# pennneutrinos/chroma

Hardware: AMD Instinct MI355X
Metric: photons/sec (propagate_hit) (higher is better)
Workload: dtype f32

## Files before the change

### chroma_amd/csrc/chroma_hip.hip

```cpp
#include <math.h>
#include <stdio.h>
#include <stdlib.h>
#include <string.h>
#include <algorithm>

#ifndef CHROMA_EXPERIMENTAL
#define CHROMA_EXPERIMENTAL 0
#endif
#ifndef CHROMA_HYBRID_RENDER
#define CHROMA_HYBRID_RENDER 1
#endif
#include "chroma_internal.h"
#include "propagate_device.h"

#include "kernel_propagate_fused.h"

#include "kernel_step_control.h"

#include "kernels_raycast_crosscheck.h"

#include "kernel_raycast_quad.h"

#include "kernel_raycast_pair.h"

// ... 60 lines not shown
    {"pair", nullptr, Cast::PAIR, 32, 4 * PAIR_WAVES_PER_EU, "CHROMA_PAIR_WAVES_PER_CU", PAIR_STACK + COOP_SPILL, SPILL_COOP, CHROMA_WALK_QUAD, false, true},
    {"literal", "exact", Cast::LITERAL, 16, 4 * QUAD_WAVES_PER_EU, "CHROMA_QUAD_WAVES_PER_CU", 0, SPILL_COOP, -1, true, true},
    {"literal_lane", nullptr, Cast::LITERAL_LANE, PROP_BLOCK, 20, "CHROMA_RAY_WAVES_PER_CU", 0, SPILL_NONE, -1, false, false},
};
static const int NWALKS = sizeof WALKS / sizeof WALKS[0];
static_assert(NWALKS == CHROMA_WALK_LITERAL_LANE + 1, "one row per CHROMA_WALK_*");

static bool walk_fits(const Walk &w, const chroma_geometry *geom)
{
    return w.stack == 0 || (geom->view.wnodes != nullptr && geom->wide_stack_need <= w.stack);
}

struct CallPlan {
    int tail_mode;
    bool counting;
    Cast cast;
    bool chain;
    bool tail_watch;
    bool tail;
    bool isect_quad;
    unsigned spill;
    int packet;
    int autosort;
};

static int make_plan(const CallState &cs, const chroma_geometry *geom, int walk, int tail, int counting, CallPlan *plan)
{
    if (walk >= NWALKS) return set_error(CHROMA_ERR_INVALID, "unknown walk mode %d", walk);
    if (tail > CHROMA_TAIL_FUSED) return set_error(CHROMA_ERR_INVALID, "unknown tail mode %d", tail);
    const int w = walk >= 0 ? walk : cs.walk;
    CallPlan p = {};
    p.tail_mode = tail >= 0 ? tail : cs.tail_mode;
    p.counting = counting >= 0 ? counting != 0 : cs.counting != 0;
    int r = w;
    while (!walk_fits(WALKS[r], geom)) {
        r = WALKS[r].fallback;
        if (w == CHROMA_WALK_PAIR && r == CHROMA_WALK_COOP) r = WALKS[r].fallback;
    }
    p.cast = WALKS[r].cast;
    p.chain = r == w && WALKS[w].chain;
    const bool fits_coop = walk_fits(WALKS[CHROMA_WALK_COOP], geom);
    p.tail_watch = p.tail_mode == CHROMA_TAIL_COOP && WALKS[w].tail;
    p.tail = p.tail_watch && fits_coop;
    p.isect_quad = fits_coop && WALKS[w].stack != 0;
    if (p.tail_mode != CHROMA_TAIL_FUSED) p.spill = WALKS[r].spill | (p.tail ? SPILL_COOP : SPILL_NONE);
    if (p.chain && p.cast == Cast::QUAD) {
        p.autosort = cs.autosort_mode;
#if CHROMA_EXPERIMENTAL
        if (geom->wide_stack_need <= PACKET_STACK) p.packet = cs.packet_mode;
#endif
    }
    *plan = p;
    return CHROMA_OK;
}

static int ensure_spill(const CallScope &scope, unsigned kinds)
{
    chroma_ctx *ctx = scope.ctx; CallState &cs = scope.state();
    const struct { SpillKind kind; uint2 **buf; size_t depth; } bufs[] = {{SPILL_COOP, &cs.coop_spill, COOP_SPILL},
                                                                          {SPILL_WIDE, &cs.wide_spill, WIDE_SPILL}};
    for (const auto &b : bufs) {
        if (!(kinds & b.kind) || *b.buf) continue;
        size_t rays = 0;
        for (const Walk &w : WALKS)
            if (w.spill == b.kind) rays = std::max(rays, (size_t)ctx->waves[(int)w.cast] * w.rays_per_wave);
        HIP_TRY(hipSetDevice(ctx->device));
        HIP_TRY(ctx_malloc(ctx, (void **)b.buf, rays * b.depth * sizeof(uint2)));
    }
    return CHROMA_OK;
}

static unsigned cast_waves(const chroma_ctx *ctx, Cast cast, long long n)
{
    const long long per = WALKS[(int)cast].rays_per_wave;
    return (unsigned)std::min<long long>((n + per - 1) / per, ctx->waves[(int)cast]);
}
// ... 54 lines not shown
namespace {
struct PropagateCall {
    const CallScope &scope; CallState &cs;
    chroma_ctx *ctx; chroma_geometry *geom;
    CallPlan plan;
    PhotonView pv; chroma_rng rng; chroma_propagate_options opt;
    uint64_t nphotons; uint32_t ncopies;
    uint32_t *in_q, *out_q;
    float4 *work_in, *work_out;
    float4 *rays, *rays_next;
    float4 *final_rec;
    uint32_t final_epoch;
    HitsOut ho;
    bool finalize;
    chroma_propagate_stats acc;
    long long n_upper;
    bool finalized;
    chroma_tracks *tracks;

    hipEvent_t *events(int step) const { return opt.time_kernels ? cs.step_events.data() + EV_PER_STEP * step : nullptr; }

    int load_working()
    {
        const unsigned blocks = (unsigned)std::min<uint64_t>((nphotons + PHYS_BLOCK - 1) / PHYS_BLOCK, (uint64_t)ctx->physics_blocks);
        int rc = scope.clear_words(W_PACKET_USE, W_PACKET_END - W_PACKET_USE); if (rc) return rc;
        uint32_t *d_order = nullptr;
        rc = propagate_order(*this, &d_order); if (rc) return rc;
        hipLaunchKernelGGL(k_load_working, dim3(blocks), dim3(PHYS_BLOCK), 0, ctx->stream, geom->view, pv, in_q, work_in,
                           (uint64_t)nphotons, ncopies, (uint32_t)(nphotons / ncopies), plan.chain ? rays : nullptr,
                           plan.packet == 2 ? cs.d_words + W_PACKET_COHERENT : nullptr, (const uint32_t *)d_order, plan.cast == Cast::LITERAL ? 1 : 0);
        if (d_order) { chroma_free(ctx, d_order); acc.reordered += nphotons; }
#if CHROMA_EXPERIMENTAL
        if (plan.packet)
            hipLaunchKernelGGL(k_packet_decide, dim3(1), dim3(1), 0, ctx->stream, cs.d_words + W_PACKET_COHERENT, cs.d_words + W_PACKET_USE,
                               (uint64_t)nphotons, plan.packet);
#endif
        HIP_TRY(hipGetLastError());
        return CHROMA_OK;
    }

    void launch_step_begin(uint32_t first_n)
    {
        hipLaunchKernelGGL(k_step_begin, dim3(1), dim3(1), 0, ctx->stream, in_q, out_q, cs.d_step,
                           tracks ? 0u : opt.use_weights ? 0xFFFFFFFFu : (uint32_t)(PROP_BLOCK * 16 * 8), first_n);
    }

    void launch_physics(int scatter_first, int fixup)
    {
        StepState *st = cs.d_step;
        float4 *chained = plan.chain ? rays_next : nullptr;
        const bool plain = geom->view.plain_optics != 0;
        bool deal = false;
#if PHYS_DEAL
        deal = plain && !final_rec;
#endif
        const int pb = deal ? PHYS_DEAL_BLOCK : PHYS_BLOCK_OF(!plain);
        unsigned blocks = (unsigned)std::min<long long>((n_upper + pb - 1) / pb, std::max<long long>(1, (long long)ctx->physics_blocks * PHYS_BLOCK / pb));
        if (fixup == 1 && plain) blocks = std::max(std::min(blocks, 64u), blocks / 8);
        DeviceCounters *pc = plan.counting ? cs.d_counters : nullptr;
#if PHYS_DEAL
        if (deal) {
            hipLaunchKernelGGL(k_physics_deal, dim3(blocks), dim3(PHYS_DEAL_BLOCK), 0, ctx->stream, geom->view, pv, st, work_in, out_q, work_out,
                               cs.hit_triangle, cs.hit_distance, rng.seed, rng.photon_id_base, opt.use_weights, scatter_first,
                               cs.retry_list, fixup, pc, chained);
            return;
        }
#endif
        const int literal_rays = fixup == 2 ? 1 : 0;
        with_bool(!plain, [&](auto FULL) {
            hipLaunchKernelGGL((k_physics<FULL>), dim3(blocks), dim3(PHYS_BLOCK_OF(FULL)), 0, ctx->stream, geom->view, pv, st, work_in, out_q,
                               work_out, cs.hit_triangle, cs.hit_distance, rng.seed, rng.photon_id_base, opt.use_weights, scatter_first,
                               cs.retry_list, fixup, pc, chained, final_rec, final_epoch, literal_rays);
        });
    }

    int launch_split_step(int scatter_first, hipEvent_t *ev, uint32_t first_n, bool packet)
    {
        if (n_upper <= 0) return CHROMA_OK;
        StepState *st = cs.d_step;
        const Cast cast = plan.cast;
        const bool exact = cast == Cast::LITERAL || cast == Cast::LITERAL_LANE;
        const dim3 block(PROP_BLOCK);
        auto record = [&](int slot) { return ev ? hipEventRecord(ev[slot], ctx->stream) : hipSuccess; };
        const unsigned rblocks = (unsigned)std::min<long long>((n_upper + PROP_BLOCK - 1) / PROP_BLOCK, 8 * 256);
        auto retry = [&](auto C) {
            hipLaunchKernelGGL((k_raycast_retry<C>), dim3(rblocks), block, 0, ctx->stream, geom->view, rays, st, cs.hit_triangle,
                               cs.hit_distance, cs.retry_list, cs.d_counters);
        };
        launch_step_begin(first_n);
        HIP_TRY(record(EV_STEP_BEGIN));
        if (!plan.chain) {
            unsigned sblocks = (unsigned)std::min<long long>((n_upper + 255) / 256, (long long)ctx->physics_blocks * 4);
            hipLaunchKernelGGL(k_ray_setup, dim3(sblocks), dim3(256), 0, ctx->stream, geom->view, work_in, st, rays,
                               cs.hit_triangle, cs.hit_distance, cs.retry_list, &st->retry, cast == Cast::LITERAL ? 1 : 0);
        }
        HIP_TRY(record(EV_PACKET_BEGIN));
        const uint32_t *skip_quad = nullptr;
#if CHROMA_EXPERIMENTAL
        if (packet) {
// ... 26 lines not shown
                                   cs.hit_distance, cs.retry_list, cs.coop_spill, cs.d_counters, ctx->coop_chunk);
                break;
            case Cast::WIDE:
                hipLaunchKernelGGL((k_raycast_wide<C>), grid, block, 0, ctx->stream, geom->view, rays, 0, st, cs.hit_triangle,
                                   cs.hit_distance, cs.retry_list, cs.wide_spill, cs.d_counters, ctx->ray_chunk);
                break;
            case Cast::PERSISTENT:
                hipLaunchKernelGGL((k_raycast_persistent<C>), grid, block, 0, ctx->stream, geom->view, rays, 0, st, cs.hit_triangle,
                                   cs.hit_distance, cs.retry_list, cs.d_counters);
                break;
            case Cast::LITERAL:
                hipLaunchKernelGGL((k_raycast_literal<C>), grid, block, 0, ctx->stream, geom->view, rays, st, cs.hit_triangle,
                                   cs.hit_distance, cs.coop_spill, cs.d_counters, ctx->coop_chunk, chained, cs.retry_list,
                                   ctx->claim_static);
                retry(C);
                break;
            case Cast::LITERAL_LANE:
                hipLaunchKernelGGL((k_raycast_retry<C, true>), grid, block, 0, ctx->stream, geom->view, rays, st, cs.hit_triangle,
                                   cs.hit_distance, cs.retry_list, cs.d_counters);
                break;
            }
        });
        HIP_TRY(record(EV_CAST_END));
        launch_physics(scatter_first, exact ? 2 : 0);
        HIP_TRY(record(EV_PHYSICS_END));
        if (!exact) {
            with_bool(plan.counting, retry);
            launch_physics(scatter_first, 1);
        }
        HIP_TRY(record(EV_STEP_END));
        HIP_TRY(hipGetLastError());
        if (plan.chain) std::swap(rays, rays_next);
        return CHROMA_OK;
    }

    int launch_tail(int nsteps, int scatter_first, hipEvent_t *ev, uint32_t first_n, bool *done)
    {
        *done = false;
        const unsigned waves = cast_waves(ctx, Cast::COOP, n_upper);
        if ((long long)waves * 8 < n_upper) return CHROMA_OK;
        launch_step_begin(first_n);
        HitsOut beside; memset(&beside, 0, sizeof beside);
        uint32_t *words = nullptr;
        if (finalize) {
            beside = ho;
            words = cs.d_words;
            int rc = scope.clear_results(); if (rc) return rc;
            if (final_rec)
                hipLaunchKernelGGL(k_mark_tail, dim3(32), dim3(256), 0, ctx->stream, in_q, final_rec, photon_tail_stamp(final_epoch));
            HIP_TRY(hipEventRecord(cs.ev_fork, ctx->stream));
        }
// ... 46 lines not shown
        }
        return CHROMA_OK;
    }

    int run_device_steps()
    {
        const int max_steps = opt.max_steps;
        HIP_TRY(hipMemsetAsync(cs.d_step, 0, sizeof(StepState), ctx->stream));
        hipLaunchKernelGGL(k_set_word, dim3(1), dim3(1), 0, ctx->stream, in_q, 1u);
        hipLaunchKernelGGL(k_set_word, dim3(1), dim3(1), 0, ctx->stream, out_q, 1u);
        int rc = load_working(); if (rc) return rc;
        const int nev = opt.time_kernels ? EV_PER_STEP * max_steps : 0;
        while ((int)cs.step_events.size() < nev) { hipEvent_t e; HIP_TRY(hipEventCreate(&e)); cs.step_events.push_back(e); }
        const long long few = (long long)PROP_BLOCK * 16 * 8;
        int step = 0, next_check = 1, tail_step = -1;
        bool done = false;
        while (step < max_steps && !done) {
            const int scatter_first = step == 0 ? opt.scatter_first : 0;
            const uint32_t first_n = step == 0 ? (uint32_t)nphotons : 0u;
            if (plan.tail && n_upper < few) {
                rc = launch_tail(max_steps - step, scatter_first, events(step), first_n, &done); if (rc) return rc;
                if (done) { tail_step = step++; break; }
            }
            rc = launch_split_step(scatter_first, events(step), first_n, step == 0 && plan.packet != 0); if (rc) return rc;
            step++;
            std::swap(in_q, out_q);
            std::swap(work_in, work_out);
            if (step == next_check && step < max_steps) {
                rc = scope.read_survivors(in_q, &n_upper); if (rc) return rc;
                if (n_upper <= 0) done = true;
                next_check = (plan.tail_watch && n_upper < 16 * few) ? step + 1 : (step < 8) ? step * 2 : step + 8;
            }
        }
        if (!done) {
            unsigned blocks = (unsigned)std::min<long long>((n_upper + 255) / 256, 4096);
            hipLaunchKernelGGL(k_store_working, dim3(std::max(blocks, 1u)), dim3(256), 0, ctx->stream, geom->view, pv, in_q, work_in);
        }
        HIP_TRY(hipMemcpyAsync(cs.h_step, cs.d_step, sizeof(StepState), hipMemcpyDeviceToHost, ctx->stream));
        HIP_TRY(hipStreamSynchronize(ctx->stream));
        acc.launches += ((const StepState *)cs.h_step)->launches;
        return opt.time_kernels ? read_step_times(step, tail_step) : CHROMA_OK;
    }

    void store_working()
    {
        const unsigned blocks = (unsigned)std::min<long long>((n_upper + 255) / 256, 4096);
        hipLaunchKernelGGL(k_store_working, dim3(std::max(blocks, 1u)), dim3(256), 0, ctx->stream, geom->view, pv, in_q, work_in);
// ... 137 lines not shown

int propagate_settings(const CallScope &scope)
{
    chroma_ctx *ctx = scope.ctx; CallState &cs = scope.state();
    hipDeviceProp_t prop;
    HIP_TRY(hipGetDeviceProperties(&prop, ctx->device));
    ctx->physics_blocks = prop.multiProcessorCount * 8;
    const char *walk = getenv("CHROMA_WALK");
    if (walk) cs.walk = CHROMA_WALK_QUAD;
    for (int w = 0; w < NWALKS; w++) {
        const Walk &row = WALKS[w];
        int per_cu = row.waves_per_cu;
        if (const char *e = getenv(row.waves_env)) per_cu = std::max(1, atoi(e));
        ctx->waves[(int)row.cast] = prop.multiProcessorCount * per_cu;
        if (walk && (!strcmp(walk, row.name) || (row.alias && !strcmp(walk, row.alias)))) cs.walk = w;
    }
#if CHROMA_EXPERIMENTAL
    if (const char *e = getenv("CHROMA_PACKET")) cs.packet_mode = !strcmp(e, "on") ? 1 : !strcmp(e, "auto") ? 2 : 0;
    if (const char *e = getenv("CHROMA_AUTOSORT")) cs.autosort_mode = !strcmp(e, "on") || !strcmp(e, "1") ? 1 : !strcmp(e, "off") || !strcmp(e, "0") ? 0 : 2;
#endif
    if (const char *e = getenv("CHROMA_RAY_CHUNK")) ctx->ray_chunk = std::max(64, atoi(e));
    if (const char *e = getenv("CHROMA_COOP_CHUNK")) ctx->coop_chunk = std::max(8, atoi(e));
    if (const char *e = getenv("CHROMA_CLAIM_STATIC")) { int big = 0, small = 0; if (sscanf(e, "%d:%d", &big, &small) < 2) small = big; ctx->claim_static = std::min(8, std::max(0, big)) | std::min(8, std::max(0, small)) << 4; }
    if (const char *e = getenv("CHROMA_TAIL"))
        cs.tail_mode = !strcmp(e, "fused") ? CHROMA_TAIL_FUSED : !strcmp(e, "split") ? CHROMA_TAIL_SPLIT : CHROMA_TAIL_COOP;
    return CHROMA_OK;
}

extern "C" {

int chroma_propagate_step(chroma_ctx *ctx, chroma_geometry *geom, int32_t first_photon, int32_t nthreads,
                          const uint32_t *d_input_queue, uint32_t *d_output_queue, chroma_rng rng,
                          const chroma_photon_arrays *photons, int32_t max_steps, int32_t use_weights,
                          int32_t scatter_first)
{
    if (!ctx || !geom) return set_error(CHROMA_ERR_INVALID, "bad argument");
    int rc = check_photons(photons, true);
    if (rc) return rc;
    if (first_photon < 0 || nthreads < 0) return set_error(CHROMA_ERR_INVALID, "negative photon range");
    if (nthreads == 0) return CHROMA_OK;
    if ((rc = check_stack(geom))) return rc;
    const CallScope scope(ctx);
    return launch_propagate(scope, scope.state().counting != 0, geom, to_view(photons), rng,
                            {first_photon, nthreads, d_input_queue, d_output_queue, max_steps, use_weights, scatter_first});
}

// ... 167 lines not shown
{
    chroma_ctx *ctx = scope.ctx; CallState &cs = scope.state();
    if (cs.final_capacity >= n) return CHROMA_OK;
    HIP_TRY(hipStreamSynchronize(ctx->stream));
    if (cs.final_rec) hipFree(cs.final_rec);
    cs.final_rec = nullptr; cs.final_capacity = 0;
    HIP_TRY(ctx_malloc(ctx, (void **)&cs.final_rec, n * 4 * sizeof(float4)));
    HIP_TRY(hipMemsetAsync(cs.final_rec, 0, n * 4 * sizeof(float4), ctx->stream));
    cs.final_capacity = n;
    cs.final_epoch = 0;
    return CHROMA_OK;
}

static int propagate_impl(chroma_ctx *ctx, chroma_geometry *geom, const chroma_photon_arrays *photons, uint64_t nphotons,
                          uint32_t ncopies, chroma_rng rng, const chroma_propagate_options &opt,
                          chroma_propagate_stats *stats, int32_t *aborted, chroma_hits_request *hr)
{
    if (!ctx || !geom) return set_error(CHROMA_ERR_INVALID, "bad argument");
    int rc = check_photons(photons, true); if (rc) return rc;
    const CallScope scope(ctx);
    CallState &cs = scope.state();
    CallPlan plan;
    rc = make_plan(cs, geom, opt.walk, opt.tail, opt.counting, &plan); if (rc) return rc;
    if (hr) {
        hr->nhits = 0;
        if (!geom->view.nsolids) return set_error(CHROMA_ERR_INVALID, "geometry has no detector channel map");
        if (hr->dst) { rc = check_photons(hr->dst, false); if (rc) return rc; }
        if ((hr->dst != nullptr) != (hr->d_channels != nullptr)) return set_error(CHROMA_ERR_INVALID, "flat hits need both dst and d_channels");
    }
    if (nphotons >= 0x7fffffffull) return set_error(CHROMA_ERR_INVALID, "at most 2^31-2 photons per call");
    if (ncopies == 0 || nphotons % ncopies) return set_error(CHROMA_ERR_INVALID, "nphotons must be a multiple of ncopies");
    if (aborted) *aborted = 0;
    const bool stepping = opt.max_steps > 0;
    if (nphotons == 0 || (!stepping && !hr)) return CHROMA_OK;
    if (stepping && (rc = check_stack(geom))) return rc;
    HIP_TRY(hipSetDevice(ctx->device));
    if (stepping) {
        rc = ensure_queues(scope, nphotons); if (rc) return rc;
        rc = ensure_spill(scope, plan.spill); if (rc) return rc;
    }
    static const bool records_always = getenv("CHROMA_FINAL_RECORDS") && atoi(getenv("CHROMA_FINAL_RECORDS")) != 0;
    const bool use_records = stepping && (hr != nullptr || records_always) && plan.tail_mode != CHROMA_TAIL_FUSED;
    if (use_records) {
        rc = ensure_final_records(scope, nphotons); if (rc) return rc;
        cs.final_epoch++;
        if (cs.final_epoch == 0u || cs.final_epoch >= 0x7FFFFFFFu) {
// ... 235 lines not shown
```

### chroma_amd/csrc/chroma_internal.h

```cpp
#pragma once
#include <hip/hip_runtime.h>
#include <stdint.h>
#include <array>
#include <map>
#include <mutex>
#include <type_traits>
#include <unordered_map>
#include <vector>

#include <rccl/rccl.h>

#include "device_common.h"

#define CHROMA_LOCAL __attribute__((visibility("hidden")))

CHROMA_LOCAL int set_error(int code, const char *fmt, ...);

#define HIP_TRY(expr)                                                                          \
    do {                                                                                       \
        hipError_t e_ = (expr);                                                                \
        if (e_ != hipSuccess)                                                                  \
            return set_error((int)e_, "%s failed: %s (%s:%d)", #expr, hipGetErrorString(e_), __FILE__, __LINE__); \
    } while (0)

// ... 3 lines not shown
    int32_t *hit_triangle = nullptr;
    float *hit_distance = nullptr;
    uint32_t *retry_list = nullptr;
    float4 *rays = nullptr;
    float4 *rays_b = nullptr;
    float4 *work_a = nullptr, *work_b = nullptr;
    float4 *final_rec = nullptr; size_t final_capacity = 0; uint32_t final_epoch = 0;
    DeviceCounters *d_counters = nullptr;
    uint32_t *d_words = nullptr;
    uint32_t *h_words = nullptr;
    StepState *d_step = nullptr;
    uint32_t *h_step = nullptr;
    std::vector<hipEvent_t> step_events;
    uint2 *wide_spill = nullptr;
    uint2 *coop_spill = nullptr;
    hipEvent_t ev_start = nullptr, ev_stop = nullptr, ev_mid = nullptr;
    hipStream_t aux_stream = nullptr;
    void *steps_scratch = nullptr; size_t steps_scratch_bytes = 0;
    hipEvent_t ev_fork = nullptr, ev_join = nullptr;
    int counting = 0;
    int tail_mode = CHROMA_TAIL_COOP;
    int autosort_mode = 0;
    int packet_mode = 0;
    int walk = CHROMA_WALK_QUAD;
};

struct chroma_ctx {
    int device;
    hipStream_t stream;
    int physics_blocks = 256 * 8;
    int waves[CHROMA_WALK_LITERAL_LANE + 1] = {};
    int ray_chunk = 256, coop_chunk = 64;
    int claim_static = 5 | 8 << 4;
    ncclComm_t comm = nullptr;
    int comm_nranks = 1, comm_rank = 0;
    uint32_t *gather_buf = nullptr;
    size_t gather_capacity = 0;
    struct PoolBlock { void *ptr; hipEvent_t ev; };
    std::mutex pool_mu;
    std::multimap<size_t, PoolBlock> pool;
    std::unordered_map<void *, size_t> live;
    std::vector<hipEvent_t> pool_events;
    size_t pool_bytes = 0, pool_limit = 0;
    uint64_t pool_hits = 0, pool_misses = 0;
    hipStream_t copy_stream = nullptr;
    std::mutex stage_mu;
// ... 119 lines not shown
```

### chroma_amd/csrc/kernel_physics.h

```cpp
#pragma once

#ifndef PHYS_BLOCK
#define PHYS_BLOCK 512
#endif
#ifndef PHYS_WAVES_PER_EU
#define PHYS_WAVES_PER_EU 4
#endif
#ifndef PHYS_SORT
#define PHYS_SORT 1
#endif
#define PHYS_CLASSES 8
#ifndef PHYS_PLAIN_WAVES_PER_EU
#define PHYS_PLAIN_WAVES_PER_EU 5
#endif
#ifndef PHYS_PLAIN_BLOCK
#define PHYS_PLAIN_BLOCK 256
#endif
#define PHYS_BLOCK_OF(FULL) ((FULL) ? PHYS_BLOCK : PHYS_PLAIN_BLOCK)
template <bool FULL>
__global__ __launch_bounds__(PHYS_BLOCK_OF(FULL)) __attribute__((amdgpu_waves_per_eu(FULL ? PHYS_WAVES_PER_EU : PHYS_PLAIN_WAVES_PER_EU))) void
k_physics(GeoView g, PhotonView pv, StepState *st, const float4 *work_in, uint32_t *output_queue, float4 *work_out,
          const int32_t *hit_triangle, const float *hit_distance, uint64_t seed, uint64_t id_base,
          int use_weights, int scatter_first, uint32_t *retry_list, int fixup, DeviceCounters *counters, float4 *rays_next,
          float4 *final_rec = nullptr, uint32_t epoch = 0u, int literal_rays = 0)
{
    constexpr int BLOCK = PHYS_BLOCK_OF(FULL);
    __shared__ uint32_t s_counts[BLOCK / WAVE + 1];
    constexpr bool SORT = FULL && (PHYS_SORT != 0);
    __shared__ uint32_t s_class_count[SORT ? BLOCK / WAVE : 1][PHYS_CLASSES];
    __shared__ int32_t s_perm[SORT ? BLOCK : 1];
    const int nthreads = fixup == 1 ? (int)st->retry : (int)st->n, renorm = (int)st->renorm, renorm_next = st->in_tail ? 0 : 1;
    unsigned long long nsteps = 0;
    for (int block_base = blockIdx.x * BLOCK; block_base < nthreads; block_base += gridDim.x * BLOCK) {
    int id = block_base + threadIdx.x;
    bool alive = false;
    uint32_t photon_id = 0;
    Photon p;
    uint32_t counter = 0;
    int last_hit_record = -1;
    int sorted_slot = (id < nthreads) ? id : -1;
    if (SORT && !fixup) {
        uint32_t cls = 0;
        if (id < nthreads) {
            const int tri0 = hit_triangle[id];
            if (tri0 >= 0) {
                const uint32_t code = g.tri_phys[2 * (size_t)tri0].w;
                const int surface = convert(0xFF & (code >> 8));
                cls = 1u + (uint32_t)min(surface + 1, PHYS_CLASSES - 2);
            }
        }
        const unsigned lane = lane_id(), wave = threadIdx.x / WAVE;
        uint32_t my_rank = 0;
#pragma unroll
        for (uint32_t c = 0; c < PHYS_CLASSES; c++) {
            const unsigned long long m = __ballot(cls == c);
            if (cls == c) my_rank = (uint32_t)__popcll(m & ((1ull << lane) - 1ull));
            if (lane == 0) s_class_count[wave][c] = (uint32_t)__popcll(m);
        }
        __syncthreads();
        static_assert(!SORT || PHYS_CLASSES * (BLOCK / WAVE) == WAVE, "one lane per (class, wave) pair");
        if (wave == 0) {
            const uint32_t c = lane / (BLOCK / WAVE), w = lane % (BLOCK / WAVE);
            const uint32_t k = s_class_count[w][c];
            uint32_t incl = k;
            for (int off = 1; off < WAVE; off <<= 1) { const uint32_t v = __shfl_up(incl, off); if ((int)lane >= off) incl += v; }
            s_class_count[w][c] = incl - k;
        }
        __syncthreads();
        s_perm[s_class_count[wave][cls] + my_rank] = (id < nthreads) ? id : -1;
        __syncthreads();
        sorted_slot = s_perm[threadIdx.x];
        __syncthreads();
    }
    if (sorted_slot >= 0) {
        const int slot = fixup == 1 ? (int)retry_list[sorted_slot] : sorted_slot;
        const float4 *w = work_in + 4 * (size_t)slot;
        const float4 w0 = w[0], w1 = w[1], w2 = w[2], w3 = w[3];
        int tri = hit_triangle[slot];
        const float hit_dist = hit_distance[slot];
        TriPhys rec = {};
        if (tri != HIT_RETRY) {
            photon_id = __float_as_uint(w3.w);
            p.position = mk3(w0.x, w0.y, w0.z);
            p.direction = mk3(w1.x, w1.y, w1.z);
            p.polarization = mk3(w2.x, w2.y, w2.z);
            if (renorm) {
                p.direction = p.direction / norm(p.direction);
                p.polarization = p.polarization / norm(p.polarization);
            }
            if (tri >= 0) rec = load_tri_phys(g, (size_t)tri);
            if (!fixup && tri >= 0) {
                const bool regular = FULL ? phys_hit_is_regular(g, rec, p.position, p.direction, hit_dist)
                                          : phys_hit_is_plainly_regular(g, rec, p.position, p.direction, hit_dist);
                if (!regular) {
                    retry_list[atomicAdd(&st->retry, 1u)] = (uint32_t)slot;
                    tri = HIT_RETRY;
                }
            }
        }
        if (tri != HIT_RETRY) {
            if (tri != HIT_NAN) nsteps++;
            p.wavelength = w0.w;
            p.time = w1.w;
            p.weight = w2.w;
            p.history = __float_as_uint(w3.x);
            p.last_hit_triangle = -1;
            p.evidx = 0;
            last_hit_record = __float_as_int(w3.z);
            cm_rng rng;
            cm_rng_init(&rng, seed, id_base + photon_id, __float_as_uint(w3.y));
            if (tri == HIT_NAN) {
                p.last_hit_triangle = last_hit_record >= 0 ? (int)g.dev_to_tri[last_hit_record] : -1;
                p.history |= CHROMA_NO_HIT | CHROMA_NAN_ABORT;
            } else {
                State s;
                if (tri >= 0) apply_hit_phys(s, p, g, rec, hit_dist);
                else apply_hit_dev(s, p, g, tri, hit_dist);
                if (tri != -1) step_after_hit<FULL>(p, s, rng, g, use_weights != 0, scatter_first);
                last_hit_record = (p.last_hit_triangle < 0) ? -1 : tri;
            }
            counter = rng.counter;
            alive = (p.history & CHROMA_TERMINAL_MASK) == 0;
            if (!alive) {
                if (final_rec) {
                    float4 *f = final_rec + 4 * (size_t)photon_id;
                    f[0] = make_float4(p.position.x, p.position.y, p.position.z, p.wavelength);
                    f[1] = make_float4(p.direction.x, p.direction.y, p.direction.z, p.time);
                    f[2] = make_float4(p.polarization.x, p.polarization.y, p.polarization.z, p.weight);
                    f[3] = make_float4(__uint_as_float(p.history), __uint_as_float(counter), __int_as_float(p.last_hit_triangle), __uint_as_float(epoch));
                } else {
                    store_photon(pv, photon_id, p, counter);
                }
            }
        }
    }
    const uint32_t at = block_queue_append<BLOCK / WAVE>(output_queue, alive, photon_id, s_counts);
    if (alive) {
        float4 *w = work_out + 4 * (size_t)(at - 1u);
        w[0] = make_float4(p.position.x, p.position.y, p.position.z, p.wavelength);
        w[1] = make_float4(p.direction.x, p.direction.y, p.direction.z, p.time);
        w[2] = make_float4(p.polarization.x, p.polarization.y, p.polarization.z, p.weight);
        w[3] = make_float4(__uint_as_float(p.history), __uint_as_float(counter), __int_as_float(last_hit_record), __uint_as_float(photon_id));
        if (rays_next) make_ray_record(g, rays_next + 4 * (size_t)(at - 1u), p.position, p.direction, renorm_next, last_hit_record, literal_rays != 0);
    }
    __syncthreads();
    }
    if (counters) {
        nsteps = wave_sum_u64(nsteps);
        if (lane_id() == 0 && nsteps) atomicAdd(&counters->photon_steps, nsteps);
    }
}
```

### chroma_amd/csrc/kernels_working_set.h

```cpp
#pragma once

__global__ __launch_bounds__(PHYS_BLOCK) void
k_load_working(GeoView g, PhotonView pv, uint32_t *queue, float4 *work, uint64_t n, uint32_t ncopies, uint32_t true_n, float4 *rays,
               uint32_t *coherence, const uint32_t *order = nullptr, int literal_rays = 0)
{
    __shared__ uint32_t s_counts[PHYS_BLOCK / WAVE + 1];
    __shared__ float4 s_stage[PHYS_BLOCK / WAVE][WAVE * 4];
#if CHROMA_EXPERIMENTAL
    uint32_t coh_yes = 0, coh_all = 0;
#endif
    for (uint64_t block_base = (uint64_t)blockIdx.x * PHYS_BLOCK; block_base < n; block_base += (uint64_t)gridDim.x * PHYS_BLOCK) {
        uint64_t j = block_base + threadIdx.x;
        bool take = false;
        uint32_t photon_id = 0, flags = 0;
        if (j < n) {
#if CHROMA_EXPERIMENTAL
            photon_id = order ? order[j] : (uint32_t)(j / ncopies) + (uint32_t)(j % ncopies) * true_n;
#else
            photon_id = (uint32_t)(j / ncopies) + (uint32_t)(j % ncopies) * true_n;
#endif
            flags = pv.flags[photon_id];
            take = (flags & CHROMA_TERMINAL_MASK) == 0;
        }
        const uint32_t at = block_queue_append<PHYS_BLOCK / WAVE>(queue, take, photon_id, s_counts);
        const unsigned long long tm = __ballot(take);
        const uint32_t nsurv = (uint32_t)__popcll(tm), rnk = (uint32_t)__popcll(tm & ((1ull << lane_id()) - 1ull));
        const uint32_t first_slot = nsurv ? (uint32_t)__shfl(at, __ffsll((long long)tm) - 1) - 1u : 0u;
        float4 *st = s_stage[threadIdx.x / WAVE];
        v3 pos = mk3(0.f, 0.f, 0.f), dir = mk3(0.f, 0.f, 1.f);
        int lh = -1;
        if (take) {
            pos = load3(pv.pos, photon_id); dir = load3(pv.dir, photon_id);
            const v3 pol = load3(pv.pol, photon_id);
            lh = pv.last_hit_triangles[photon_id];
            lh = (lh >= 0 && (uint32_t)lh < g.ntriangles) ? (int)g.tri_to_dev[lh] : -1;
            const Photon p = {pos, dir, pol, pv.wavelengths[photon_id], pv.t[photon_id], pv.weights[photon_id], flags, -1, 0u};
            PhotonRecord(p, pv.rng_counters[photon_id], lh, photon_id).store(st + 4 * rnk);
        }
        __builtin_amdgcn_wave_barrier();
        for (uint32_t q = lane_id(); q < 4u * nsurv; q += WAVE) work[4 * (size_t)first_slot + q] = st[q];
        __builtin_amdgcn_wave_barrier();
        if (rays) {
            if (take) make_ray_record(g, st + 4 * rnk, pos, dir, 1, lh, literal_rays != 0);
            __builtin_amdgcn_wave_barrier();
            for (uint32_t q = lane_id(); q < 4u * nsurv; q += WAVE) rays[4 * (size_t)first_slot + q] = st[q];
            __builtin_amdgcn_wave_barrier();
        }
        if (take) {
#if CHROMA_EXPERIMENTAL
            if (coherence) {
                const unsigned long long m = __ballot(true);
                const int first = __ffsll((long long)m) - 1;
                const float px = __shfl(pos.x, first), py = __shfl(pos.y, first), pz = __shfl(pos.z, first);
                const float qx = __shfl(dir.x, first), qy = __shfl(dir.y, first), qz = __shfl(dir.z, first);
                const float d2 = dir.x * dir.x + dir.y * dir.y + dir.z * dir.z, q2 = qx * qx + qy * qy + qz * qz;
                const float c = dir.x * qx + dir.y * qy + dir.z * qz;
                const bool near = fabsf(pos.x - px) + fabsf(pos.y - py) + fabsf(pos.z - pz) < 1.0f && c > 0.0f && c * c > 0.9975f * d2 * q2;
                const unsigned long long ok = __ballot(near);
                if ((int)lane_id() == first && __popcll(m) >= 32) { coh_all++; coh_yes += (ok == m) ? 1u : 0u; }
            }
#endif
        }
        __syncthreads();
    }
#if CHROMA_EXPERIMENTAL
    if (coherence) {
        if (coh_all) { atomicAdd(&coherence[1], coh_all); if (coh_yes) atomicAdd(&coherence[0], coh_yes); }
    }
#endif
}

__global__ void k_store_working(GeoView g, PhotonView pv, const uint32_t *queue, const float4 *work)
{
    const uint32_t n = queue[0] - 1u;
    for (uint32_t slot = blockIdx.x * blockDim.x + threadIdx.x; slot < n; slot += gridDim.x * blockDim.x) {
        const float4 *w = work + 4 * (size_t)slot;
        const float4 w0 = w[0], w1 = w[1], w2 = w[2], w3 = w[3];
        const uint32_t photon_id = __float_as_uint(w3.w);
        const int rec = __float_as_int(w3.z);
        store3(pv.pos, photon_id, mk3(w0.x, w0.y, w0.z));
        store3(pv.dir, photon_id, mk3(w1.x, w1.y, w1.z));
        store3(pv.pol, photon_id, mk3(w2.x, w2.y, w2.z));
        pv.wavelengths[photon_id] = w0.w;
        pv.t[photon_id] = w1.w;
// ... 7 lines not shown
```

Baseline: 897.8 million.

## Read first-step photon state directly from arrays instead of staging working set

Adds a k_physics_first kernel variant that, on step zero, reads photon state straight from the SoA photon arrays via the input queue rather than from a packed working buffer. k_load_working then skips writing the working records when this path is on, so the initial pass avoids one full write and read of the 64-byte-per-photon buffer. k_load_working also batches several rounds per block, doing one queue atomic per chunk instead of one per round. The cost is gathered, uncoalesced reads in the first physics step and duplicated kernel code through a shared body header.

```diff
diff --git a/chroma_amd/csrc/chroma_hip.hip b/chroma_amd/csrc/chroma_hip.hip
--- a/chroma_amd/csrc/chroma_hip.hip
+++ b/chroma_amd/csrc/chroma_hip.hip
@@ -106,6 +106,7 @@
     unsigned spill;
     int packet;
     int autosort;
+    bool first_from_arrays;
 };
 
 static int make_plan(const CallState &cs, const chroma_geometry *geom, int walk, int tail, int counting, CallPlan *plan)
@@ -136,6 +137,14 @@
     }
     *plan = p;
     return CHROMA_OK;
+}
+
+static void plan_first_step(CallPlan &plan, const CallState &cs, const chroma_propagate_options &opt, uint64_t nphotons)
+{
+    const uint64_t few = (uint64_t)PROP_BLOCK * 16 * 8;
+    const bool starts_in_tail = opt.use_weights || (plan.tail && nphotons < few);
+    plan.first_from_arrays = cs.first_from_arrays && plan.tail_mode != CHROMA_TAIL_FUSED && plan.chain &&
+                             !starts_in_tail && !plan.packet && !plan.autosort && !CHROMA_EXPERIMENTAL;
 }
 
 static int ensure_spill(const CallScope &scope, unsigned kinds)
@@ -236,11 +245,13 @@
 
     int load_working()
     {
-        const unsigned blocks = (unsigned)std::min<uint64_t>((nphotons + PHYS_BLOCK - 1) / PHYS_BLOCK, (uint64_t)ctx->physics_blocks);
+        const uint64_t chunk = (uint64_t)PHYS_BLOCK * LOAD_ROUNDS;
+        const unsigned blocks = (unsigned)std::min<uint64_t>((nphotons + chunk - 1) / chunk, (uint64_t)ctx->physics_blocks);
         int rc = scope.clear_words(W_PACKET_USE, W_PACKET_END - W_PACKET_USE); if (rc) return rc;
         uint32_t *d_order = nullptr;
         rc = propagate_order(*this, &d_order); if (rc) return rc;
-        hipLaunchKernelGGL(k_load_working, dim3(blocks), dim3(PHYS_BLOCK), 0, ctx->stream, geom->view, pv, in_q, work_in,
+        hipLaunchKernelGGL(k_load_working, dim3(blocks), dim3(PHYS_BLOCK), 0, ctx->stream, geom->view, pv, in_q,
+                           plan.first_from_arrays ? nullptr : work_in,
                            (uint64_t)nphotons, ncopies, (uint32_t)(nphotons / ncopies), plan.chain ? rays : nullptr,
                            plan.packet == 2 ? cs.d_words + W_PACKET_COHERENT : nullptr, (const uint32_t *)d_order, plan.cast == Cast::LITERAL ? 1 : 0);
         if (d_order) { chroma_free(ctx, d_order); acc.reordered += nphotons; }
@@ -259,7 +270,7 @@
                            tracks ? 0u : opt.use_weights ? 0xFFFFFFFFu : (uint32_t)(PROP_BLOCK * 16 * 8), first_n);
     }
 
-    void launch_physics(int scatter_first, int fixup)
+    void launch_physics(int scatter_first, int fixup, bool first)
     {
         StepState *st = cs.d_step;
         float4 *chained = plan.chain ? rays_next : nullptr;
@@ -281,6 +292,14 @@
         }
 #endif
         const int literal_rays = fixup == 2 ? 1 : 0;
+        if (first) {
+            with_bool(!plain, [&](auto FULL) {
+                hipLaunchKernelGGL((k_physics_first<FULL>), dim3(blocks), dim3(PHYS_BLOCK_OF(FULL)), 0, ctx->stream, geom->view, pv, st,
+                                   (const uint32_t *)in_q, out_q, work_out, cs.hit_triangle, cs.hit_distance, rng.seed, rng.photon_id_base,
+                                   opt.use_weights, scatter_first, cs.retry_list, fixup, pc, chained, final_rec, final_epoch, literal_rays);
+            });
+            return;
+        }
         with_bool(!plain, [&](auto FULL) {
             hipLaunchKernelGGL((k_physics<FULL>), dim3(blocks), dim3(PHYS_BLOCK_OF(FULL)), 0, ctx->stream, geom->view, pv, st, work_in, out_q,
                                work_out, cs.hit_triangle, cs.hit_distance, rng.seed, rng.photon_id_base, opt.use_weights, scatter_first,
@@ -288,7 +307,7 @@
         });
     }
 
-    int launch_split_step(int scatter_first, hipEvent_t *ev, uint32_t first_n, bool packet)
+    int launch_split_step(int scatter_first, hipEvent_t *ev, uint32_t first_n, bool packet, bool first = false)
     {
         if (n_upper <= 0) return CHROMA_OK;
         StepState *st = cs.d_step;
@@ -361,11 +380,11 @@
             }
         });
         HIP_TRY(record(EV_CAST_END));
-        launch_physics(scatter_first, exact ? 2 : 0);
+        launch_physics(scatter_first, exact ? 2 : 0, first);
         HIP_TRY(record(EV_PHYSICS_END));
         if (!exact) {
             with_bool(plan.counting, retry);
-            launch_physics(scatter_first, 1);
+            launch_physics(scatter_first, 1, first);
         }
         HIP_TRY(record(EV_STEP_END));
         HIP_TRY(hipGetLastError());
@@ -458,7 +477,8 @@
                 rc = launch_tail(max_steps - step, scatter_first, events(step), first_n, &done); if (rc) return rc;
                 if (done) { tail_step = step++; break; }
             }
-            rc = launch_split_step(scatter_first, events(step), first_n, step == 0 && plan.packet != 0); if (rc) return rc;
+            rc = launch_split_step(scatter_first, events(step), first_n, step == 0 && plan.packet != 0, step == 0 && plan.first_from_arrays);
+            if (rc) return rc;
             step++;
             std::swap(in_q, out_q);
             std::swap(work_in, work_out);
@@ -642,6 +662,7 @@
     if (const char *e = getenv("CHROMA_RAY_CHUNK")) ctx->ray_chunk = std::max(64, atoi(e));
     if (const char *e = getenv("CHROMA_COOP_CHUNK")) ctx->coop_chunk = std::max(8, atoi(e));
     if (const char *e = getenv("CHROMA_CLAIM_STATIC")) { int big = 0, small = 0; if (sscanf(e, "%d:%d", &big, &small) < 2) small = big; ctx->claim_static = std::min(8, std::max(0, big)) | std::min(8, std::max(0, small)) << 4; }
+    if (const char *e = getenv("CHROMA_FIRST_STEP")) cs.first_from_arrays = strcmp(e, "working") != 0;
     if (const char *e = getenv("CHROMA_TAIL"))
         cs.tail_mode = !strcmp(e, "fused") ? CHROMA_TAIL_FUSED : !strcmp(e, "split") ? CHROMA_TAIL_SPLIT : CHROMA_TAIL_COOP;
     return CHROMA_OK;
@@ -855,6 +876,7 @@
     CallState &cs = scope.state();
     CallPlan plan;
     rc = make_plan(cs, geom, opt.walk, opt.tail, opt.counting, &plan); if (rc) return rc;
+    plan_first_step(plan, cs, opt, nphotons);
     if (hr) {
         hr->nhits = 0;
         if (!geom->view.nsolids) return set_error(CHROMA_ERR_INVALID, "geometry has no detector channel map");
diff --git a/chroma_amd/csrc/chroma_internal.h b/chroma_amd/csrc/chroma_internal.h
--- a/chroma_amd/csrc/chroma_internal.h
+++ b/chroma_amd/csrc/chroma_internal.h
@@ -49,6 +49,7 @@
     int tail_mode = CHROMA_TAIL_COOP;
     int autosort_mode = 0;
     int packet_mode = 0;
+    int first_from_arrays = 1;
     int walk = CHROMA_WALK_QUAD;
 };
 
diff --git a/chroma_amd/csrc/kernel_physics.h b/chroma_amd/csrc/kernel_physics.h
--- a/chroma_amd/csrc/kernel_physics.h
+++ b/chroma_amd/csrc/kernel_physics.h
@@ -24,129 +24,19 @@
           int use_weights, int scatter_first, uint32_t *retry_list, int fixup, DeviceCounters *counters, float4 *rays_next,
           float4 *final_rec = nullptr, uint32_t epoch = 0u, int literal_rays = 0)
 {
-    constexpr int BLOCK = PHYS_BLOCK_OF(FULL);
-    __shared__ uint32_t s_counts[BLOCK / WAVE + 1];
-    constexpr bool SORT = FULL && (PHYS_SORT != 0);
-    __shared__ uint32_t s_class_count[SORT ? BLOCK / WAVE : 1][PHYS_CLASSES];
-    __shared__ int32_t s_perm[SORT ? BLOCK : 1];
-    const int nthreads = fixup == 1 ? (int)st->retry : (int)st->n, renorm = (int)st->renorm, renorm_next = st->in_tail ? 0 : 1;
-    unsigned long long nsteps = 0;
-    for (int block_base = blockIdx.x * BLOCK; block_base < nthreads; block_base += gridDim.x * BLOCK) {
-    int id = block_base + threadIdx.x;
-    bool alive = false;
-    uint32_t photon_id = 0;
-    Photon p;
-    uint32_t counter = 0;
-    int last_hit_record = -1;
-    int sorted_slot = (id < nthreads) ? id : -1;
-    if (SORT && !fixup) {
-        uint32_t cls = 0;
-        if (id < nthreads) {
-            const int tri0 = hit_triangle[id];
-            if (tri0 >= 0) {
-                const uint32_t code = g.tri_phys[2 * (size_t)tri0].w;
-                const int surface = convert(0xFF & (code >> 8));
-                cls = 1u + (uint32_t)min(surface + 1, PHYS_CLASSES - 2);
-            }
-        }
-        const unsigned lane = lane_id(), wave = threadIdx.x / WAVE;
-        uint32_t my_rank = 0;
-#pragma unroll
-        for (uint32_t c = 0; c < PHYS_CLASSES; c++) {
-            const unsigned long long m = __ballot(cls == c);
-            if (cls == c) my_rank = (uint32_t)__popcll(m & ((1ull << lane) - 1ull));
-            if (lane == 0) s_class_count[wave][c] = (uint32_t)__popcll(m);
-        }
-        __syncthreads();
-        static_assert(!SORT || PHYS_CLASSES * (BLOCK / WAVE) == WAVE, "one lane per (class, wave) pair");
-        if (wave == 0) {
-            const uint32_t c = lane / (BLOCK / WAVE), w = lane % (BLOCK / WAVE);
-            const uint32_t k = s_class_count[w][c];
-            uint32_t incl = k;
-            for (int off = 1; off < WAVE; off <<= 1) { const uint32_t v = __shfl_up(incl, off); if ((int)lane >= off) incl += v; }
-            s_class_count[w][c] = incl - k;
-        }
-        __syncthreads();
-        s_perm[s_class_count[wave][cls] + my_rank] = (id < nthreads) ? id : -1;
-        __syncthreads();
-        sorted_slot = s_perm[threadIdx.x];
-        __syncthreads();
-    }
-    if (sorted_slot >= 0) {
-        const int slot = fixup == 1 ? (int)retry_list[sorted_slot] : sorted_slot;
-        const float4 *w = work_in + 4 * (size_t)slot;
-        const float4 w0 = w[0], w1 = w[1], w2 = w[2], w3 = w[3];
-        int tri = hit_triangle[slot];
-        const float hit_dist = hit_distance[slot];
-        TriPhys rec = {};
-        if (tri != HIT_RETRY) {
-            photon_id = __float_as_uint(w3.w);
-            p.position = mk3(w0.x, w0.y, w0.z);
-            p.direction = mk3(w1.x, w1.y, w1.z);
-            p.polarization = mk3(w2.x, w2.y, w2.z);
-            if (renorm) {
-                p.direction = p.direction / norm(p.direction);
-                p.polarization = p.polarization / norm(p.polarization);
-            }
-            if (tri >= 0) rec = load_tri_phys(g, (size_t)tri);
-            if (!fixup && tri >= 0) {
-                const bool regular = FULL ? phys_hit_is_regular(g, rec, p.position, p.direction, hit_dist)
-                                          : phys_hit_is_plainly_regular(g, rec, p.position, p.direction, hit_dist);
-                if (!regular) {
-                    retry_list[atomicAdd(&st->retry, 1u)] = (uint32_t)slot;
-                    tri = HIT_RETRY;
-                }
-            }
-        }
-        if (tri != HIT_RETRY) {
-            if (tri != HIT_NAN) nsteps++;
-            p.wavelength = w0.w;
-            p.time = w1.w;
-            p.weight = w2.w;
-            p.history = __float_as_uint(w3.x);
-            p.last_hit_triangle = -1;
-            p.evidx = 0;
-            last_hit_record = __float_as_int(w3.z);
-            cm_rng rng;
-            cm_rng_init(&rng, seed, id_base + photon_id, __float_as_uint(w3.y));
-            if (tri == HIT_NAN) {
-                p.last_hit_triangle = last_hit_record >= 0 ? (int)g.dev_to_tri[last_hit_record] : -1;
-                p.history |= CHROMA_NO_HIT | CHROMA_NAN_ABORT;
-            } else {
-                State s;
-                if (tri >= 0) apply_hit_phys(s, p, g, rec, hit_dist);
-                else apply_hit_dev(s, p, g, tri, hit_dist);
-                if (tri != -1) step_after_hit<FULL>(p, s, rng, g, use_weights != 0, scatter_first);
-                last_hit_record = (p.last_hit_triangle < 0) ? -1 : tri;
-            }
-            counter = rng.counter;
-            alive = (p.history & CHROMA_TERMINAL_MASK) == 0;
-            if (!alive) {
-                if (final_rec) {
-                    float4 *f = final_rec + 4 * (size_t)photon_id;
-                    f[0] = make_float4(p.position.x, p.position.y, p.position.z, p.wavelength);
-                    f[1] = make_float4(p.direction.x, p.direction.y, p.direction.z, p.time);
-                    f[2] = make_float4(p.polarization.x, p.polarization.y, p.polarization.z, p.weight);
-                    f[3] = make_float4(__uint_as_float(p.history), __uint_as_float(counter), __int_as_float(p.last_hit_triangle), __uint_as_float(epoch));
-                } else {
-                    store_photon(pv, photon_id, p, counter);
-                }
-            }
-        }
-    }
-    const uint32_t at = block_queue_append<BLOCK / WAVE>(output_queue, alive, photon_id, s_counts);
-    if (alive) {
-        float4 *w = work_out + 4 * (size_t)(at - 1u);
-        w[0] = make_float4(p.position.x, p.position.y, p.position.z, p.wavelength);
-        w[1] = make_float4(p.direction.x, p.direction.y, p.direction.z, p.time);
-        w[2] = make_float4(p.polarization.x, p.polarization.y, p.polarization.z, p.weight);
-        w[3] = make_float4(__uint_as_float(p.history), __uint_as_float(counter), __int_as_float(last_hit_record), __uint_as_float(photon_id));
-        if (rays_next) make_ray_record(g, rays_next + 4 * (size_t)(at - 1u), p.position, p.direction, renorm_next, last_hit_record, literal_rays != 0);
-    }
-    __syncthreads();
-    }
-    if (counters) {
-        nsteps = wave_sum_u64(nsteps);
-        if (lane_id() == 0 && nsteps) atomicAdd(&counters->photon_steps, nsteps);
-    }
+#define PHYSICS_FROM_ARRAYS 0
+#include "kernel_physics_body.h"
+#undef PHYSICS_FROM_ARRAYS
 }
+
+template <bool FULL>
+__global__ __launch_bounds__(PHYS_BLOCK_OF(FULL)) __attribute__((amdgpu_waves_per_eu(FULL ? PHYS_WAVES_PER_EU : PHYS_PLAIN_WAVES_PER_EU))) void
+k_physics_first(GeoView g, PhotonView pv, StepState *st, const uint32_t *input_queue, uint32_t *output_queue, float4 *work_out,
+                const int32_t *hit_triangle, const float *hit_distance, uint64_t seed, uint64_t id_base,
+                int use_weights, int scatter_first, uint32_t *retry_list, int fixup, DeviceCounters *counters, float4 *rays_next,
+                float4 *final_rec = nullptr, uint32_t epoch = 0u, int literal_rays = 0)
+{
+#define PHYSICS_FROM_ARRAYS 1
+#include "kernel_physics_body.h"
+#undef PHYSICS_FROM_ARRAYS
+}
diff --git a/chroma_amd/csrc/kernel_physics_body.h b/chroma_amd/csrc/kernel_physics_body.h
--- /dev/null
+++ b/chroma_amd/csrc/kernel_physics_body.h
@@ -0,0 +1,137 @@
+    constexpr int BLOCK = PHYS_BLOCK_OF(FULL);
+    __shared__ uint32_t s_counts[BLOCK / WAVE + 1];
+    constexpr bool SORT = FULL && (PHYS_SORT != 0);
+    __shared__ uint32_t s_class_count[SORT ? BLOCK / WAVE : 1][PHYS_CLASSES];
+    __shared__ int32_t s_perm[SORT ? BLOCK : 1];
+    const int nthreads = fixup == 1 ? (int)st->retry : (int)st->n, renorm = (int)st->renorm, renorm_next = st->in_tail ? 0 : 1;
+    unsigned long long nsteps = 0;
+    for (int block_base = blockIdx.x * BLOCK; block_base < nthreads; block_base += gridDim.x * BLOCK) {
+    int id = block_base + threadIdx.x;
+    bool alive = false;
+    uint32_t photon_id = 0;
+    Photon p;
+    uint32_t counter = 0;
+    int last_hit_record = -1;
+    int sorted_slot = (id < nthreads) ? id : -1;
+    if (SORT && !fixup) {
+        uint32_t cls = 0;
+        if (id < nthreads) {
+            const int tri0 = hit_triangle[id];
+            if (tri0 >= 0) {
+                const uint32_t code = g.tri_phys[2 * (size_t)tri0].w;
+                const int surface = convert(0xFF & (code >> 8));
+                cls = 1u + (uint32_t)min(surface + 1, PHYS_CLASSES - 2);
+            }
+        }
+        const unsigned lane = lane_id(), wave = threadIdx.x / WAVE;
+        uint32_t my_rank = 0;
+#pragma unroll
+        for (uint32_t c = 0; c < PHYS_CLASSES; c++) {
+            const unsigned long long m = __ballot(cls == c);
+            if (cls == c) my_rank = (uint32_t)__popcll(m & ((1ull << lane) - 1ull));
+            if (lane == 0) s_class_count[wave][c] = (uint32_t)__popcll(m);
+        }
+        __syncthreads();
+        static_assert(!SORT || PHYS_CLASSES * (BLOCK / WAVE) == WAVE, "one lane per (class, wave) pair");
+        if (wave == 0) {
+            const uint32_t c = lane / (BLOCK / WAVE), w = lane % (BLOCK / WAVE);
+            const uint32_t k = s_class_count[w][c];
+            uint32_t incl = k;
+            for (int off = 1; off < WAVE; off <<= 1) { const uint32_t v = __shfl_up(incl, off); if ((int)lane >= off) incl += v; }
+            s_class_count[w][c] = incl - k;
+        }
+        __syncthreads();
+        s_perm[s_class_count[wave][cls] + my_rank] = (id < nthreads) ? id : -1;
+        __syncthreads();
+        sorted_slot = s_perm[threadIdx.x];
+        __syncthreads();
+    }
+    if (sorted_slot >= 0) {
+        const int slot = fixup == 1 ? (int)retry_list[sorted_slot] : sorted_slot;
+#if PHYSICS_FROM_ARRAYS
+        const uint32_t queued_id = input_queue[1 + slot];
+        const v3 pos0 = load3(pv.pos, queued_id), dir0 = load3(pv.dir, queued_id), pol0 = load3(pv.pol, queued_id);
+        int lh0 = pv.last_hit_triangles[queued_id];
+        lh0 = (lh0 >= 0 && (uint32_t)lh0 < g.ntriangles) ? (int)g.tri_to_dev[lh0] : -1;
+        const float4 w0 = make_float4(pos0.x, pos0.y, pos0.z, pv.wavelengths[queued_id]);
+        const float4 w1 = make_float4(dir0.x, dir0.y, dir0.z, pv.t[queued_id]);
+        const float4 w2 = make_float4(pol0.x, pol0.y, pol0.z, pv.weights[queued_id]);
+        const float4 w3 = make_float4(__uint_as_float(pv.flags[queued_id]), __uint_as_float(pv.rng_counters[queued_id]), __int_as_float(lh0),
+                                      __uint_as_float(queued_id));
+#else
+        const float4 *w = work_in + 4 * (size_t)slot;
+        const float4 w0 = w[0], w1 = w[1], w2 = w[2], w3 = w[3];
+#endif
+        int tri = hit_triangle[slot];
+        const float hit_dist = hit_distance[slot];
+        TriPhys rec = {};
+        if (tri != HIT_RETRY) {
+            photon_id = __float_as_uint(w3.w);
+            p.position = mk3(w0.x, w0.y, w0.z);
+            p.direction = mk3(w1.x, w1.y, w1.z);
+            p.polarization = mk3(w2.x, w2.y, w2.z);
+            if (renorm) {
+                p.direction = p.direction / norm(p.direction);
+                p.polarization = p.polarization / norm(p.polarization);
+            }
+            if (tri >= 0) rec = load_tri_phys(g, (size_t)tri);
+            if (!fixup && tri >= 0) {
+                const bool regular = FULL ? phys_hit_is_regular(g, rec, p.position, p.direction, hit_dist)
+                                          : phys_hit_is_plainly_regular(g, rec, p.position, p.direction, hit_dist);
+                if (!regular) {
+                    retry_list[atomicAdd(&st->retry, 1u)] = (uint32_t)slot;
+                    tri = HIT_RETRY;
+                }
+            }
+        }
+        if (tri != HIT_RETRY) {
+            if (tri != HIT_NAN) nsteps++;
+            p.wavelength = w0.w;
+            p.time = w1.w;
+            p.weight = w2.w;
+            p.history = __float_as_uint(w3.x);
+            p.last_hit_triangle = -1;
+            p.evidx = 0;
+            last_hit_record = __float_as_int(w3.z);
+            cm_rng rng;
+            cm_rng_init(&rng, seed, id_base + photon_id, __float_as_uint(w3.y));
+            if (tri == HIT_NAN) {
+                p.last_hit_triangle = last_hit_record >= 0 ? (int)g.dev_to_tri[last_hit_record] : -1;
+                p.history |= CHROMA_NO_HIT | CHROMA_NAN_ABORT;
+            } else {
+                State s;
+                if (tri >= 0) apply_hit_phys(s, p, g, rec, hit_dist);
+                else apply_hit_dev(s, p, g, tri, hit_dist);
+                if (tri != -1) step_after_hit<FULL>(p, s, rng, g, use_weights != 0, scatter_first);
+                last_hit_record = (p.last_hit_triangle < 0) ? -1 : tri;
+            }
+            counter = rng.counter;
+            alive = (p.history & CHROMA_TERMINAL_MASK) == 0;
+            if (!alive) {
+                if (final_rec) {
+                    float4 *f = final_rec + 4 * (size_t)photon_id;
+                    f[0] = make_float4(p.position.x, p.position.y, p.position.z, p.wavelength);
+                    f[1] = make_float4(p.direction.x, p.direction.y, p.direction.z, p.time);
+                    f[2] = make_float4(p.polarization.x, p.polarization.y, p.polarization.z, p.weight);
+                    f[3] = make_float4(__uint_as_float(p.history), __uint_as_float(counter), __int_as_float(p.last_hit_triangle), __uint_as_float(epoch));
+                } else {
+                    store_photon(pv, photon_id, p, counter);
+                }
+            }
+        }
+    }
+    const uint32_t at = block_queue_append<BLOCK / WAVE>(output_queue, alive, photon_id, s_counts);
+    if (alive) {
+        float4 *w = work_out + 4 * (size_t)(at - 1u);
+        w[0] = make_float4(p.position.x, p.position.y, p.position.z, p.wavelength);
+        w[1] = make_float4(p.direction.x, p.direction.y, p.direction.z, p.time);
+        w[2] = make_float4(p.polarization.x, p.polarization.y, p.polarization.z, p.weight);
+        w[3] = make_float4(__uint_as_float(p.history), __uint_as_float(counter), __int_as_float(last_hit_record), __uint_as_float(photon_id));
+        if (rays_next) make_ray_record(g, rays_next + 4 * (size_t)(at - 1u), p.position, p.direction, renorm_next, last_hit_record, literal_rays != 0);
+    }
+    __syncthreads();
+    }
+    if (counters) {
+        nsteps = wave_sum_u64(nsteps);
+        if (lane_id() == 0 && nsteps) atomicAdd(&counters->photon_steps, nsteps);
+    }
diff --git a/chroma_amd/csrc/kernels_working_set.h b/chroma_amd/csrc/kernels_working_set.h
--- a/chroma_amd/csrc/kernels_working_set.h
+++ b/chroma_amd/csrc/kernels_working_set.h
@@ -1,45 +1,82 @@
 #pragma once
 
+#define LOAD_ROUNDS 4
 __global__ __launch_bounds__(PHYS_BLOCK) void
 k_load_working(GeoView g, PhotonView pv, uint32_t *queue, float4 *work, uint64_t n, uint32_t ncopies, uint32_t true_n, float4 *rays,
                uint32_t *coherence, const uint32_t *order = nullptr, int literal_rays = 0)
 {
-    __shared__ uint32_t s_counts[PHYS_BLOCK / WAVE + 1];
-    __shared__ float4 s_stage[PHYS_BLOCK / WAVE][WAVE * 4];
+    constexpr int NW = PHYS_BLOCK / WAVE;
+    __shared__ uint32_t s_counts[LOAD_ROUNDS][NW];
+    __shared__ uint32_t s_base;
+    __shared__ float4 s_stage[NW][WAVE * 4];
 #if CHROMA_EXPERIMENTAL
     uint32_t coh_yes = 0, coh_all = 0;
 #endif
-    for (uint64_t block_base = (uint64_t)blockIdx.x * PHYS_BLOCK; block_base < n; block_base += (uint64_t)gridDim.x * PHYS_BLOCK) {
-        uint64_t j = block_base + threadIdx.x;
-        bool take = false;
-        uint32_t photon_id = 0, flags = 0;
+    const uint64_t chunk = (uint64_t)PHYS_BLOCK * LOAD_ROUNDS;
+    for (uint64_t chunk_base = (uint64_t)blockIdx.x * chunk; chunk_base < n; chunk_base += (uint64_t)gridDim.x * chunk) {
+        uint32_t round_flags[LOAD_ROUNDS];
+#pragma unroll
+        for (int r = 0; r < LOAD_ROUNDS; r++) {
+            const uint64_t j = chunk_base + (uint64_t)r * PHYS_BLOCK + threadIdx.x;
+            round_flags[r] = CHROMA_TERMINAL_MASK;
+            if (j < n) {
+#if CHROMA_EXPERIMENTAL
+                round_flags[r] = pv.flags[order ? order[j] : (uint32_t)(j / ncopies) + (uint32_t)(j % ncopies) * true_n];
+#else
+                round_flags[r] = pv.flags[(uint32_t)(j / ncopies) + (uint32_t)(j % ncopies) * true_n];
+#endif
+            }
+        }
+#pragma unroll
+        for (int r = 0; r < LOAD_ROUNDS; r++) {
+            const unsigned long long m = __ballot((round_flags[r] & CHROMA_TERMINAL_MASK) == 0);
+            if (lane_id() == 0) s_counts[r][threadIdx.x / WAVE] = (uint32_t)__popcll(m);
+        }
+        __syncthreads();
+        if (threadIdx.x == 0) {
+            uint32_t total = 0;
+            for (int r = 0; r < LOAD_ROUNDS; r++)
+                for (int w = 0; w < NW; w++) { const uint32_t c = s_counts[r][w]; s_counts[r][w] = total; total += c; }
+            s_base = total ? atomicAdd(queue, total) : 0u;
+        }
+        __syncthreads();
+#pragma unroll 1
+        for (int r = 0; r < LOAD_ROUNDS; r++) {
+        const uint64_t j = chunk_base + (uint64_t)r * PHYS_BLOCK + threadIdx.x;
+        uint32_t flags = round_flags[0];
+#pragma unroll
+        for (int k = 1; k < LOAD_ROUNDS; k++) flags = r == k ? round_flags[k] : flags;
+        const bool take = (flags & CHROMA_TERMINAL_MASK) == 0;
+        uint32_t photon_id = 0;
         if (j < n) {
 #if CHROMA_EXPERIMENTAL
             photon_id = order ? order[j] : (uint32_t)(j / ncopies) + (uint32_t)(j % ncopies) * true_n;
 #else
             photon_id = (uint32_t)(j / ncopies) + (uint32_t)(j % ncopies) * true_n;
 #endif
-            flags = pv.flags[photon_id];
-            take = (flags & CHROMA_TERMINAL_MASK) == 0;
         }
-        const uint32_t at = block_queue_append<PHYS_BLOCK / WAVE>(queue, take, photon_id, s_counts);
+        v3 pos = mk3(0.f, 0.f, 0.f), dir = mk3(0.f, 0.f, 1.f);
+        int lh = -1;
         const unsigned long long tm = __ballot(take);
         const uint32_t nsurv = (uint32_t)__popcll(tm), rnk = (uint32_t)__popcll(tm & ((1ull << lane_id()) - 1ull));
-        const uint32_t first_slot = nsurv ? (uint32_t)__shfl(at, __ffsll((long long)tm) - 1) - 1u : 0u;
+        const uint32_t first_slot = s_base + s_counts[r][threadIdx.x / WAVE] - 1u;
+        if (take) queue[first_slot + 1u + rnk] = photon_id;
         float4 *st = s_stage[threadIdx.x / WAVE];
-        v3 pos = mk3(0.f, 0.f, 0.f), dir = mk3(0.f, 0.f, 1.f);
-        int lh = -1;
         if (take) {
             pos = load3(pv.pos, photon_id); dir = load3(pv.dir, photon_id);
-            const v3 pol = load3(pv.pol, photon_id);
             lh = pv.last_hit_triangles[photon_id];
             lh = (lh >= 0 && (uint32_t)lh < g.ntriangles) ? (int)g.tri_to_dev[lh] : -1;
-            const Photon p = {pos, dir, pol, pv.wavelengths[photon_id], pv.t[photon_id], pv.weights[photon_id], flags, -1, 0u};
-            PhotonRecord(p, pv.rng_counters[photon_id], lh, photon_id).store(st + 4 * rnk);
         }
-        __builtin_amdgcn_wave_barrier();
-        for (uint32_t q = lane_id(); q < 4u * nsurv; q += WAVE) work[4 * (size_t)first_slot + q] = st[q];
-        __builtin_amdgcn_wave_barrier();
+        if (work) {
+            if (take) {
+                const v3 pol = load3(pv.pol, photon_id);
+                const Photon p = {pos, dir, pol, pv.wavelengths[photon_id], pv.t[photon_id], pv.weights[photon_id], flags, -1, 0u};
+                PhotonRecord(p, pv.rng_counters[photon_id], lh, photon_id).store(st + 4 * rnk);
+            }
+            __builtin_amdgcn_wave_barrier();
+            for (uint32_t q = lane_id(); q < 4u * nsurv; q += WAVE) work[4 * (size_t)first_slot + q] = st[q];
+            __builtin_amdgcn_wave_barrier();
+        }
         if (rays) {
             if (take) make_ray_record(g, st + 4 * rnk, pos, dir, 1, lh, literal_rays != 0);
             __builtin_amdgcn_wave_barrier();
@@ -60,6 +97,7 @@
                 if ((int)lane_id() == first && __popcll(m) >= 32) { coh_all++; coh_yes += (ok == m) ? 1u : 0u; }
             }
 #endif
+        }
         }
         __syncthreads();
     }
```

Result: no change. 905.6 million (median of 6 runs) (+0.9%).
